# jhuldr/BrainFM

Hardware: AMD Instinct MI355X
Metric: voxels/sec whole-volume multi-task inference, 256^3 tiled (higher is better)
Workload: dtype f16x3-split (fp32-grade); 1 GPU; 256^3 volume, reference tiling win160/stride80 -> 27 tiles, UNet3D f64 x6 levels, 9 heads (69 ch), fused tail + deformed atlas + on-device stitch of 17 keys; stitched_keys=17, mfma_passes=3, submission=hipGraph replay per tile shape, parallelism=tiles sharded over 1 rank(s), gather to rank 0, tiles_in_flight_per_gpu=2

## Files before the change

### brainfm_amd/_lib.py

```python
import ctypes as C
import os

_HERE = os.path.dirname(os.path.abspath(__file__))
LIB_PATH = os.path.join(_HERE, "libbrainfm_hip.so")

ERR = {0: "BFM_OK", -1: "BFM_E_ARG", -2: "BFM_E_SHAPE", -3: "BFM_E_WORKSPACE", -4: "BFM_E_LAUNCH"}

ROLE_PLAIN, ROLE_CT, ROLE_BIAS_LOG, ROLE_SEG, ROLE_DIST, ROLE_SR, ROLE_PATHOL = range(7)
(EW_EXP, EW_AFFINE, EW_CLAMP, EW_CLAMP_MIN, EW_GAMMA, EW_SIGMOID, EW_DIV, EW_NONZERO, EW_SUB_DIV, EW_GE,
 EW_NAN_TO_NUM) = range(11)
(EW_ADD, EW_MUL, EW_MUL_EXP, EW_AXPY_CLAMP0, EW_AXPY, EW_DIV2, EW_ZERO_WHERE_ZERO) = range(7)


class BfmError(RuntimeError):
    pass


class Upsample(C.Structure):
    _fields_ = [("d", C.c_int), ("h", C.c_int), ("w", C.c_int),
                ("mapD", C.c_void_p), ("mapH", C.c_void_p), ("mapW", C.c_void_p),
                ("repD", C.c_void_p), ("repH", C.c_void_p), ("repW", C.c_void_p)]


CLASS_STATS_BLOCKS = 1024
# ... 94 lines not shown
    "bfm_conv3x3x3_upfold_batch_workspace": (_Z, [_I, _I, _I, _I, _I, _I]),
    "bfm_conv3x3x3_upfold_batch": (_I, [_P, _I, _I, _I, _I, _I, _P, _P, _P, _I, _P, _I, _I, _I, _P, _P, _Z, _I, _P]),
    "bfm_conv3x3x3_tap_batch_workspace": (_Z, [_I, _I, _I, _I]),
    "bfm_conv3x3x3_tap_batch": (_I, [_P, _I, _I, _I, _P, _P, _P, _I, _P, _I, _I, _I, _I, _I, _P, _Z, _I, _P]),
    "bfm_tap_sum_rows": (_I, [_I, _I]),
    "bfm_tap_sum_batch": (_I, [_P, _I, _I, _I, _I, _P, _I, _F, _I, _I, _P, _P, _P]),
    "bfm_moment_rows_bytes": (_Z, [_I, _I]),
    "bfm_conv3x3x3_mfma_rows": (_I, [_I, _I, _I, _I, _I, C.POINTER(_I)]),
    "bfm_conv3x3x3_mfma_ex": (_I, [_P, _I, _P, _I, _I, _I, _I, _UP, _P, _P, _P, _I, _P, _I, _I, _F, _I,
                                   C.POINTER(_I), _P, _P, _Z, _P, _P]),
    "bfm_conv3x3x3_mfma_batch_workspace": (_Z, [_I, _I, _I, _I, _I, _I, _I]),
    "bfm_conv3x3x3_mfma_batch": (_I, [_P, _I, _P, _I, _I, _I, _I, _I, _UP, _P, _P, _P, _I, _P, _I, _I, _F, _I,
                                      C.POINTER(_I), _P, _P, _Z, _P, _I, _P]),
    "bfm_gn_stats_batch_workspace": (_Z, [_I, _I, _I, _I, _I, _I, _UP]),
    "bfm_gn_stats_batch": (_I, [_P, _I, _P, _I, _I, _I, _I, _I, _UP, _P, _P, _I, _F, _P, _P, _P, _P, _Z, _P]),
    "bfm_gn_stats_rows_batch": (_I, [_P, _I, _I, _P, _I, _I, C.c_double, _L, _I, _P, _P, _I, _F, _P, _P, _P, _P]),
    "bfm_conv3x3x3_stem_rows": (_I, [_I, _I, _I]),
    "bfm_conv3x3x3_stem_ex": (_I, [_P, _I, _I, _I, _P, _P, _P, _P, _I, _F, _P, _P, _P]),
    "bfm_conv3x3x3_stem_mc_ex": (_I, [_P, _I, _I, _I, _I, _P, _P, _P, _P, _I, _F, _P, _P, _P]),
    "bfm_gn_stats_rows_workspace": (_Z, [_I, _I, _I, _I]),
    "bfm_gn_stats_plan": (_I, [_I, _L, _I, C.POINTER(_I), C.POINTER(_I), C.POINTER(_L), C.POINTER(_I)]),
    "bfm_gn_stats_rows_route": (_I, [_I, _I, _I, _I, _I, _I]),
    "bfm_gn_stats_rows": (_I, [_P, _I, _I, _P, _I, _I, C.c_double, _L, _P, _P, _I, _F, _P, _P, _P, _P, _Z, _P, _P]),
    "bfm_gn_stats_rows_sliced": (_I, [_P, _I, _I, _I, _I, _P, _I, _I, _I, _I, C.c_double, _L, _P, _P, _I, _F, _P, _P, _P, _P, _Z,
                                      _P, _P]),
    "bfm_gn_stats_rows_train": (_I, [_P, _I, _I, _P, _I, _I, C.c_double, _L, _P, _P, _I, _F, _P, _P, _P, _P, _P, _P, _Z, _P, _P]),
    "bfm_crop3d": (_I, [_P, _I, _I, _I, _I, _I, _I, _I, _I, _I, _P, _P]),
    "bfm_pack_conv_weights_wino4_bytes": (_Z, [_I, _I, _I]),
    "bfm_pack_conv_weights_wino4": (_I, [_P, _I, _I, _F, _I, _P, C.POINTER(_I), _P]),
    "bfm_conv3x3x3_wino4_rows": (_I, [_I, _I, _I, _I]),
    "bfm_conv3x3x3_wino4_box": (_I, [_I, _I, _I, _I, _P]),
    "bfm_conv3x3x3_wino4_masked_workspace": (_Z, [_I, _I, _I, _I]),
    "bfm_conv3x3x3_wino4_uniform_scratch": (_Z, [_I]),
    "bfm_conv3x3x3_wino4_uniform": (_I, [_P, _I, _I, _I, _I, _P, _P, _P, _I, _P, _I, _I, _F, _I, _I, _P, _P, _P, _P, _P]),
    "bfm_conv3x3x3_wino4_uniform_keep": (_I, [_P, _I, _I, _I, _I, _P, _P, _P, _I, _P, _I, _I, _F, _I, _I, _P, _P, _P, _P, _P, _P]),
    "bfm_conv3x3x3_wino4": (_I, [_P, _I, _I, _I, _I, _P, _P, _P, _I, _P, _I, _I, _F, _I, _I, _P, _P, _P]),
    "bfm_conv3x3x3_wino4_batch": (_I, [_P, _I, _I, _I, _I, _I, _P, _P, _P, _I, _P, _I, _I, _F, _I, _I, _P, _P, _I, _P]),
    "bfm_conv3x3x3_wino_b5_rows": (_I, [_I, _I, _I, _I]),
    "bfm_conv3x3x3_wino_b5_splitk": (_I, [_I, _I, _I, _I, _I]),
    "bfm_conv3x3x3_wino_b5_workspace": (_Z, [_I, _I, _I, _I, _I, _I]),
    "bfm_conv3x3x3_wino_b5_batch": (_I, [_P, _I, _I, _I, _I, _I, _P, _P, _P, _I, _P, _I, _I, _F, _I, _I, _P, _P, _I, _P, _Z,
                                         _P]),
    "bfm_conv3x3x3_wino4_masked": (_I, [_P, _I, _I, _I, _I, _P, _P, _P, _I, _P, _I, _I, _F, _I, _I, _P, _P, _P, _Z, _P]),
    "bfm_permute_flip3d": (_I, [_P, _I, _I, _I, C.POINTER(_I), C.POINTER(_I), _P, _P]),
    "bfm_bbox_nonzero": (_I, [_P, _I, _I, _I, _F, _P, _P]),
    "bfm_mean_lastdim": (_I, [_P, _L, _I, _P, _P]),
    "bfm_pack_conv_weights_wino_bytes": (_Z, [_I, _I, _I]),
    "bfm_pack_conv_weights_wino": (_I, [_P, _I, _I, _F, _I, _P, C.POINTER(_I), _P]),
    "bfm_bspline3_prefilter_axis": (_I, [_P, _I, _I, _I, _I, _I, _F, _F, _P, _F, _F, _F, _I, _P]),
    "bfm_bspline3_resample_axis": (_I, [_P, _I, _I, _I, _I, _P, _I, _I, _P, _P]),
    "bfm_conv3x3x3_wino_rows": (_I, [_I, _I, _I, _I]),
    "bfm_conv3x3x3_wino_ex": (_I, [_P, _I, _I, _I, _I, _P, _P, _P, _I, _P, _I, _I, _F, _I, _I, _P, _P, _P]),
    "bfm_conv3x3x3_wino_box": (_I, [_I, _I, _I, _I, _P]),
    "bfm_uniform_boxes": (_I, [_P, _I, _I, _I, _I, _I, _P, _P]),
    "bfm_uniform_boxes_level": (_I, [_P, _I, _I, _I, _I, _I, _I, _P, _P]),
    "bfm_uniform_boxes_levels": (_I, [_P, _I, _I, _I, _I, C.POINTER(_I), C.POINTER(_I), _I, C.POINTER(_P), _P, _P]),
    "bfm_uniform_boxes_bytes": (_Z, [_I, _I, _I, _I]),
    "bfm_uniform_fill": (_I, [_P, _I, _I, _I, _I, _I, _P, _P]),
    "bfm_conv3x3x3_wino_uniform_scratch": (_Z, [_I]),
    "bfm_conv3x3x3_wino_uniform": (_I, [_P, _I, _I, _I, _I, _P, _P, _P, _I, _P, _I, _I, _F, _I, _I, _P, _P, _P, _P, _P]),
    "bfm_conv3x3x3_wino_pool_ok": (_I, [_I, _I, _I, _I]),
    "bfm_conv3x3x3_wino_pool": (_I, [_P, _I, _I, _I, _I, _P, _P, _P, _I, _P, _I, _I, _F, _I, _I, _P, _P, _P, _P, _P]),
    "bfm_conv3x3x3_wino_uniform_pool": (_I, [_P, _I, _I, _I, _I, _P, _P, _P, _I, _P, _I, _I, _F, _I, _I, _P, _P, _P, _P, _P, _P,
                                             _P]),
    "bfm_conv3x3x3_wino_masked_workspace": (_Z, [_I, _I, _I, _I]),
    "bfm_conv3x3x3_wino_masked": (_I, [_P, _I, _I, _I, _I, _P, _P, _P, _I, _P, _I, _I, _F, _I, _I, _P, _P, _P, _Z, _P]),
# ... 259 lines not shown
```

### brainfm_amd/csrc/conv3d_wino4.hip

```cpp
#include "wino_shared.h"
#include <cstdlib>
#include <type_traits>

namespace {

typedef _Float16 half8 __attribute__((ext_vector_type(8)));
typedef float floatx16 __attribute__((ext_vector_type(16)));
typedef __fp16 fp16x2_t __attribute__((ext_vector_type(2)));

constexpr int KC = 16;
constexpr int NPOS = 6;
constexpr int NTHR = 256;
constexpr int NRG = NTHR / 32;
constexpr int MLD = 33;

struct W4Params {
    const float* A;
    int CA, D, H, W;
    const float *scale, *shift, *bound;
    int G;
    const uint4* wp;
    int wexp, Cout;
    float slope;
    float* out;
    int accum;
    int TD, TH, TW, HT, QW;
    int qw_shift, thq_shift;
    int nTy, nTx, nMt, NT, KCN;
    int npos_lds, plane_stride;
    double *rsum, *rsq;
    float *rmn, *rmx;
    const int* list;
    const int* list_n;
// ... 350 lines not shown
        if (p.rsum != nullptr) {
            double* ls = reinterpret_cast<double*>(lds + (size_t)NPOS * 64 * MLD * sizeof(float));
            double* lq = ls + NRG * 32;
            float* lmn = reinterpret_cast<float*>(lq + NRG * 32);
            float* lmx = lmn + NRG * 32;
            ls[rg * 32 + col] = (double)fs; lq[rg * 32 + col] = (double)fq;
            lmn[rg * 32 + col] = fmn; lmx[rg * 32 + col] = fmx;
            __syncthreads();
            if (tid < 32) {
                double Ssum = 0.0, Q = 0.0;
                float MN = INFINITY, MX = -INFINITY;
#pragma unroll
                for (int r = 0; r < NRG; ++r) {
                    Ssum += ls[r * 32 + tid]; Q += lq[r * 32 + tid];
                    MN = fminf(MN, lmn[r * 32 + tid]); MX = fmaxf(MX, lmx[r * 32 + tid]);
                }
                const size_t o = (size_t)mt * p.Cout + nt * 64 + nb * 32 + tid;
                p.rsum[o] = Ssum; p.rsq[o] = Q; p.rmn[o] = MN; p.rmx[o] = MX;
            }
        }
    }
}

template <int NPASS>
__global__ void __launch_bounds__(NTHR, 2) conv_wino4(const W4Params p) { conv_wino4_body<NPASS, 0>(p); }
template <int NPASS>
__global__ void __launch_bounds__(NTHR, 2) conv_wino4_masked(const W4Params p) { conv_wino4_body<NPASS, 1>(p); }

constexpr int DB_TD = 8, DB_TH = 8, DB_HT = 10, DB_NROW = 100;
constexpr int DB_PLANE = DB_NROW * 16;
constexpr int DB_RAWROW = 6 * 64;
constexpr int DB_RAW = DB_NROW * DB_RAWROW;
constexpr int DB_NDMA = DB_NROW / 2;
constexpr int DB_NDMA_WAVE = (DB_NDMA + 3) / 4;

template <bool LO>
__device__ __forceinline__ void split_store4_mix(const float (&t)[4], unsigned char* dp, int plane_stride) {
    const fp16x2_t h01 = __builtin_amdgcn_cvt_pkrtz(t[0], t[1]);
    const fp16x2_t h23 = __builtin_amdgcn_cvt_pkrtz(t[2], t[3]);
    uint2 hv;
    hv.x = __builtin_bit_cast(unsigned, h01);
    hv.y = __builtin_bit_cast(unsigned, h23);
    *reinterpret_cast<uint2*>(dp) = hv;
    if constexpr (LO) {
        uint2 lv;
        asm("v_fma_mixlo_f16 %0, %1, -1.0, %2 op_sel_hi:[1,0,0]" : "=v"(lv.x) : "v"(hv.x), "v"(t[0]));
        asm("v_fma_mixhi_f16 %0, %1, -1.0, %2 op_sel:[1,0,0] op_sel_hi:[1,0,0]" : "+v"(lv.x) : "v"(hv.x), "v"(t[1]));
        asm("v_fma_mixlo_f16 %0, %1, -1.0, %2 op_sel_hi:[1,0,0]" : "=v"(lv.y) : "v"(hv.y), "v"(t[2]));
        asm("v_fma_mixhi_f16 %0, %1, -1.0, %2 op_sel:[1,0,0] op_sel_hi:[1,0,0]" : "+v"(lv.y) : "v"(hv.y), "v"(t[3]));
        *reinterpret_cast<uint2*>(dp + plane_stride) = lv;
    }
}

template <int NPASS, int MODE, int ABL = 0>
__device__ __forceinline__ void conv_wino4d_body(const W4Params& pin) {
    W4Params p = pin;
    constexpr bool LIST = MODE != 0;
    constexpr bool UNI = MODE == 3;
    constexpr bool BY_FLAG = MODE == 2 || MODE == 3;
    constexpr int NPL = (NPASS == 3) ? 2 : 1;
    constexpr int NF = 2 * NPL;
    constexpr int NWF = 3 * NPL;
    constexpr int RAW_OFF = 2 * NPOS * NPL * DB_PLANE;
    extern __shared__ __attribute__((aligned(16))) unsigned char lds[];

    const int tid = threadIdx.x;
    const int lane = tid & 63;
    const int wv = __builtin_amdgcn_readfirstlane(tid >> 6);
    const int posA = wv;
    const int posB = 4 + (wv >> 1), nbB = wv & 1;
    const int l32 = lane & 31, khalf = lane >> 5;
#ifdef BFM_W4_ABLATE
    if (p.dbg_sleep > 0 && blockIdx.x < 512) {
        unsigned hwid;
        asm volatile("s_getreg_b32 %0, hwreg(HW_REG_HW_ID)" : "=s"(hwid));
        if (hwid & 1)
            for (int i = 0; i < p.dbg_sleep; ++i) __builtin_amdgcn_s_sleep(16);
    }
#endif
    int item;
    {
        const int nblk = LIST ? p.list_n[0] * p.NT : p.nMt * p.NT;
        const int bid = blockIdx.x;
        if (LIST && bid >= nblk) return;
        const int q = nblk >> 3, r = nblk & 7;
        const int xcd = bid & 7, idx = bid >> 3;
        item = (xcd < r ? xcd * (q + 1) : r * (q + 1) + (xcd - r) * q) + idx;
    }
    const int mt = LIST ? p.list[item / p.NT] : item / p.NT;
    const int nt = item % p.NT;
    int mtl = mt;
    if (!LIST && p.nMtS > 0) {
        const int smp = mt / p.nMtS;
        mtl = mt - smp * p.nMtS;
        p.A += smp * p.sA;
        p.out += smp * p.sO;
        p.scale += smp * p.saff;
        p.shift += smp * p.saff;
        p.bound += smp * p.G;
    }
    const int tx = mtl % p.nTx;
    const int ty = (mtl / p.nTx) % p.nTy;
    const int tz = mtl / (p.nTx * p.nTy);
    const int z0 = tz * DB_TD, y0 = ty * DB_TH, x0 = tx * 4;
    int cls = 0;
    if constexpr (BY_FLAG) cls = __builtin_amdgcn_readfirstlane((int)p.uni_flags[mt]);
    const bool rep = MODE == 2 && cls != 0;
    float4* const ybuf = BY_FLAG && cls ? reinterpret_cast<float4*>(p.uni_acc) + ((size_t)(cls - 1) * p.NT + nt) * (2 * 8 * NTHR) + tid
                                        : nullptr;
    bool store = true;
    if constexpr (UNI) {
        if (p.uni_need != nullptr) {
            store = p.uni_need[mt] != 0;
            if (!store && p.uni_keep != nullptr) store = p.uni_keep[((int64_t)z0 * p.H + y0) * p.W + x0] != 0.f;
        }
    }

    float bmax = 0.f;
    for (int g = 0; g < p.G; ++g) bmax = fmaxf(bmax, p.bound[g]);
    int aexp = 0;
    if (bmax > 0.f && bmax < INFINITY) {
        int ex;
        (void)frexpf(bmax, &ex);
        aexp = 10 - ex;
        aexp = aexp > 60 ? 60 : (aexp < -60 ? -60 : aexp);
    }
    const float a_scale = ldexpf(1.0f, aexp);
    const float dq = ldexpf(1.0f, -(aexp + p.wexp));

    floatx16 acc[2][2];
    floatx16 accB[2];
    if constexpr (!UNI) {
    int a_off[4];
#pragma unroll
    for (int u = 0; u < 4; ++u) {
        const int pos = u < 2 ? posA : posB, mb = u & 1;
        const int pr = row_perm(l32);
        const int d = mb * 2 + (pr >> 4) + 4 * ((pr & 15) >> 3), h = pr & 7;
        a_off[u] = ((pos * 2 + khalf) * NPL) * DB_PLANE + (d * DB_HT + h) * 16;
    }

    const int q4 = tid & 3;
    int msk[2];
#pragma unroll
    for (int it = 0; it < 2; ++it) {
        const int r = (tid >> 2) + 64 * it;
        msk[it] = -1;
        if (r < DB_NROW) {
            const int hz = r / DB_HT, hy = r - hz * DB_HT;
            const int gz = z0 + hz - 1, gy = y0 + hy - 1;
            int m = 0;
            if (gz >= 0 && gz < p.D && gy >= 0 && gy < p.H) {
#pragma unroll
                for (int i = 0; i < 6; ++i)
                    if (x0 - 1 + i >= 0 && x0 - 1 + i < p.W) m |= 1 << i;
            }
            msk[it] = m;
        }
    }
    const bool inner = z0 >= 1 && z0 + DB_TD < p.D && y0 >= 1 && y0 + DB_TH < p.H && x0 >= 1 && x0 + 4 < p.W;
    const int st_plane = ((q4 >> 1) * NPL) * DB_PLANE + (q4 & 1) * 8;

    const int slot = lane >> 2;
    const int sb = slot >= 6 ? 1 : 0;
    int gxc = x0 + (slot - 6 * sb) - 1;
    gxc = gxc < 0 ? 0 : (gxc > p.W - 1 ? p.W - 1 : gxc);
    const int lane_el = gxc * p.CA + (lane & 3) * 4;
    const bool dma_lane = slot < 12;
    const unsigned raw_lds = (unsigned)(__UINTPTR_TYPE__)((__attribute__((address_space(3))) unsigned char*)(lds + RAW_OFF));
    const int zs = z0 > 0 ? z0 - 1 : 0;
    const float* slab = p.A + (int64_t)zs * p.H * p.W * p.CA;
    auto issue_dma = [&](int kc) __attribute__((always_inline)) {
        if constexpr ((ABL & 8) != 0) return;
        if (dma_lane) {
            int wvo = wv;
            asm volatile("" : "+s"(wvo));
#pragma unroll
            for (int n = 0; n < DB_NDMA_WAVE; ++n) {
                const int i = wvo + 4 * n;
                if (n < DB_NDMA_WAVE - 1 || i < DB_NDMA) {
                    const int hz = i / 5, hp = i - 5 * hz;
                    int gz = z0 + hz - 1;
                    gz = gz < 0 ? 0 : (gz > p.D - 1 ? p.D - 1 : gz);
                    int gy0 = y0 + 2 * hp - 1, gy1 = gy0 + 1;
                    gy0 = gy0 < 0 ? 0 : (gy0 > p.H - 1 ? p.H - 1 : gy0);
                    gy1 = gy1 > p.H - 1 ? p.H - 1 : gy1;
                    const unsigned ro0 = (unsigned)((((gz - zs) * p.H + gy0) * p.W) * p.CA);
                    const unsigned ro1 = (unsigned)((((gz - zs) * p.H + gy1) * p.W) * p.CA);
                    const unsigned vo = ((sb ? ro1 : ro0) + (unsigned)lane_el) * 4u;
                    const unsigned la = raw_lds + (unsigned)(i * (2 * DB_RAWROW));
                    asm volatile("s_mov_b32 m0, %2\n\ts_nop 0\n\tglobal_load_lds_dwordx4 %0, %1" ::"v"(vo), "s"(slab + kc * KC), "s"(la)
                                 : "memory");
                }
            }
        }
    };

#pragma unroll
    for (int u = 0; u < 2; ++u) {
#pragma unroll
        for (int i = 0; i < 16; ++i) { acc[u][0][i] = 0.f; acc[u][1][i] = 0.f; accB[u][i] = 0.f; }
    }

    const int S = p.KCN * 9;
    const uint4* wbA = p.wp + (size_t)(nt * NPOS + posA) * S * (NF * 64) + lane;
    const uint4* wbB = p.wp + (size_t)(nt * NPOS + posB) * S * (NF * 64) + nbB * (NPL * 64) + lane;
    uint4 wq[3][NWF];
    auto fetch = [&](int s, uint4 (&dst)[NWF]) __attribute__((always_inline)) {
        if constexpr ((ABL & 1) != 0) { if (s > 2) return; }
        const int sc = s < S ? s : S - 1;
#pragma unroll
        for (int f = 0; f < NF; ++f) dst[f] = wbA[(size_t)sc * (NF * 64) + f * 64];
#pragma unroll
        for (int f = 0; f < NPL; ++f) dst[NF + f] = wbB[(size_t)sc * (NF * 64) + f * 64];
    };
    issue_dma(0);
    fetch(0, wq[0]);
    fetch(1, wq[1]);
    half8 a_abl[4][NPL];
    if constexpr ((ABL & 2) != 0) {
#pragma unroll
        for (int u = 0; u < 4; ++u)
#pragma unroll
            for (int hl = 0; hl < NPL; ++hl)
#pragma unroll
                for (int j = 0; j < 8; ++j) a_abl[u][hl][j] = (_Float16)(0.01f * (float)((lane * 7 + u * 3 + hl * 5 + j) % 61) - 0.3f);
    }

    for (int kc = 0; kc < p.KCN; ++kc) {
        const int c0 = kc * KC;
        const float4 sc4 = *reinterpret_cast<const float4*>(p.scale + c0 + q4 * 4);
        const float4 sh4 = *reinterpret_cast<const float4*>(p.shift + c0 + q4 * 4);
        const float sc[4] = {sc4.x * a_scale, sc4.y * a_scale, sc4.z * a_scale, sc4.w * a_scale};
        const float sh[4] = {sh4.x * a_scale, sh4.y * a_scale, sh4.z * a_scale, sh4.w * a_scale};
        __builtin_amdgcn_s_waitcnt(0x0F70);
        __syncthreads();
#pragma unroll
        for (int it = 0; it < 2; ++it) {
            if (msk[it] < 0) continue;
            if constexpr ((ABL & 4) != 0) continue;
            const int r = (tid >> 2) + 64 * it;
            const float4* rp = reinterpret_cast<const float4*>(
                __builtin_assume_aligned(lds + RAW_OFF + r * DB_RAWROW + q4 * 16, 16));
            float4 v[6];
#pragma unroll
            for (int i = 0; i < 6; ++i) v[i] = rp[i * 4];
            float dd[6][4];
            if (inner) {
#pragma unroll
                for (int i = 0; i < 6; ++i) {
                    const float y[4] = {v[i].x, v[i].y, v[i].z, v[i].w};
#pragma unroll
                    for (int c = 0; c < 4; ++c) dd[i][c] = fmaf(y[c], sc[c], sh[c]);
                }
            } else {
#pragma unroll
                for (int i = 0; i < 6; ++i) {
                    const bool ok = msk[it] & (1 << i);
                    const float y[4] = {v[i].x, v[i].y, v[i].z, v[i].w};
#pragma unroll
                    for (int c = 0; c < 4; ++c) {
                        const float a = fmaf(y[c], sc[c], sh[c]);
                        dd[i][c] = ok ? a : 0.f;
                    }
                }
            }
            unsigned char* dst = lds + st_plane + r * 16;
            float t[6][4];
#pragma unroll
            for (int c = 0; c < 4; ++c) {
                const float d0 = dd[0][c], d1 = dd[1][c], d2 = dd[2][c], d3 = dd[3][c], d4 = dd[4][c], d5 = dd[5][c];
                const float a = fmaf(-4.f, d2, d4);
                const float b = fmaf(-4.f, d1, d3);
                const float cc = d4 - d2;
// ... 43 lines not shown
                    for (int nb = 0; nb < 2; ++nb) {
                        const half8 bhi = __builtin_bit_cast(half8, wq[cur][nb * NPL]);
                        if constexpr (NPASS == 3) {
                            const half8 blo = __builtin_bit_cast(half8, wq[cur][nb * NPL + 1]);
                            acc[u][nb] = __builtin_amdgcn_mfma_f32_32x32x16_f16(a[1], bhi, acc[u][nb], 0, 0, 0);
                            acc[u][nb] = __builtin_amdgcn_mfma_f32_32x32x16_f16(a[0], blo, acc[u][nb], 0, 0, 0);
                        }
                        acc[u][nb] = __builtin_amdgcn_mfma_f32_32x32x16_f16(a[0], bhi, acc[u][nb], 0, 0, 0);
                    }
                } else {
                    const half8 bhi = __builtin_bit_cast(half8, wq[cur][NF]);
                    if constexpr (NPASS == 3) {
                        const half8 blo = __builtin_bit_cast(half8, wq[cur][NF + 1]);
                        accB[u - 2] = __builtin_amdgcn_mfma_f32_32x32x16_f16(a[1], bhi, accB[u - 2], 0, 0, 0);
                        accB[u - 2] = __builtin_amdgcn_mfma_f32_32x32x16_f16(a[0], blo, accB[u - 2], 0, 0, 0);
                    }
                    accB[u - 2] = __builtin_amdgcn_mfma_f32_32x32x16_f16(a[0], bhi, accB[u - 2], 0, 0, 0);
                }
            }
        }
    }

    }

    if constexpr ((ABL & 16) != 0) {
        float sm = 0.f;
#pragma unroll
        for (int u = 0; u < 2; ++u)
#pragma unroll
            for (int i = 0; i < 16; ++i) sm += acc[u][0][i] + acc[u][1][i] + accB[u][i];
        if (sm == 12345.678f) p.out[tid] = sm;
        return;
    }
    float* m = reinterpret_cast<float*>(lds);
    const int col = tid & 31, rg = tid >> 5;
    const bool interior = z0 + DB_TD <= p.D && y0 + DB_TH <= p.H && x0 + 4 <= p.W;
    int un[4];
#pragma unroll
    for (int c = 0; c < 4; ++c) un[c] = row_unperm(16 * (c >> 1) + 8 * (c & 1) + rg);
    const unsigned off_t = (unsigned)((rg * p.W) * p.Cout + col);
#pragma unroll
    for (int nb = 0; nb < 2; ++nb) {
        if constexpr (!UNI && (ABL & 256) == 0) {
        __syncthreads();
#pragma unroll
        for (int u = 0; u < 2; ++u) {
            float* mw = m + (posA * 64 + u * 32 + khalf * 4) * MLD + l32;
#pragma unroll
            for (int i = 0; i < 16; ++i)
                mw[((i >> 2) * 8 + (i & 3)) * MLD] = acc[u][nb][i];
        }
        if (nbB == nb) {
#pragma unroll
            for (int u = 0; u < 2; ++u) {
                float* mw = m + (posB * 64 + u * 32 + khalf * 4) * MLD + l32;
#pragma unroll
                for (int i = 0; i < 16; ++i)
                    mw[((i >> 2) * 8 + (i & 3)) * MLD] = accB[u][i];
            }
        }
        __syncthreads();
        } else if (nb == 1 && p.rsum != nullptr) __syncthreads();
        float fs = 0.f, fq = 0.f, fmn = INFINITY, fmx = -INFINITY;
        float* ob = p.out + nt * 64 + nb * 32 + ((int64_t)(z0 * p.H + y0) * p.W + x0) * p.Cout;
        if constexpr ((ABL & 512) != 0) ob = p.out + nt * 64 + nb * 32 + (mt & 127) * 16384;
        const float* mc = m + col;
        if (interior) {
// ... 46 lines not shown
#pragma unroll 2
            for (int it = 0; it < 8; ++it) {
                if (z0 + it >= p.D) break;
                float* o = ob + (int64_t)it * p.H * p.W * p.Cout;
                float y[4];
                if constexpr (UNI) {
                    const float4 yy = ybuf[(nb * 8 + it) * NTHR];
                    y[0] = yy.x; y[1] = yy.y; y[2] = yy.z; y[3] = yy.w;
                } else {
                    const int qr = 32 * ((it & 3) >> 1) + row_unperm(16 * (it & 1) + 8 * (it >> 2) + rg);
                    const float* mr = mc + qr * MLD;
                    const float m0 = mr[0 * 64 * MLD], m1 = mr[1 * 64 * MLD], m2 = mr[2 * 64 * MLD];
                    const float m3 = mr[3 * 64 * MLD], m4 = mr[4 * 64 * MLD], m5 = mr[5 * 64 * MLD];
                    const float s1 = m1 + m2, d1 = m1 - m2, s2 = m3 + m4, d2 = m3 - m4;
                    y[0] = ((m0 + s1) + s2) * dq;
                    y[1] = fmaf(2.f, d2, d1) * dq;
                    y[2] = fmaf(4.f, s2, s1) * dq;
                    y[3] = (fmaf(8.f, d2, d1) + m5) * dq;
                    if (MODE == 2 && rep) ybuf[(nb * 8 + it) * NTHR] = make_float4(y[0], y[1], y[2], y[3]);
                }
#pragma unroll
                for (int k = 0; k < 4; ++k) {
                    if (x0 + k < p.W) {
                        float r = y[k];
                        if (p.accum) r = r + o[off_t + (unsigned)(k * p.Cout)];
                        r = r >= 0.f ? r : r * p.slope;
                        if (!UNI || store) o[off_t + (unsigned)(k * p.Cout)] = r;
                        fs += r; fq = fmaf(r, r, fq); fmn = fminf(fmn, r); fmx = fmaxf(fmx, r);
                    }
                }
            }
        }
        if (p.rsum != nullptr) {
            double* ls = reinterpret_cast<double*>(lds + (UNI ? (size_t)0 : (size_t)NPOS * 64 * MLD * sizeof(float)));
            double* lq = ls + NRG * 32;
            float* lmn = reinterpret_cast<float*>(lq + NRG * 32);
            float* lmx = lmn + NRG * 32;
            ls[rg * 32 + col] = (double)fs; lq[rg * 32 + col] = (double)fq;
            lmn[rg * 32 + col] = fmn; lmx[rg * 32 + col] = fmx;
            __syncthreads();
            if (tid < 32) {
                double Ssum = 0.0, Q = 0.0;
                float MN = INFINITY, MX = -INFINITY;
#pragma unroll
                for (int r = 0; r < NRG; ++r) {
                    Ssum += ls[r * 32 + tid]; Q += lq[r * 32 + tid];
                    MN = fminf(MN, lmn[r * 32 + tid]); MX = fmaxf(MX, lmx[r * 32 + tid]);
                }
                const size_t o = (size_t)mt * p.Cout + nt * 64 + nb * 32 + tid;
                p.rsum[o] = Ssum; p.rsq[o] = Q; p.rmn[o] = MN; p.rmx[o] = MX;
            }
        }
    }
}

template <int NPASS>
__global__ void __launch_bounds__(NTHR, 2) conv_wino4d(const W4Params p) { conv_wino4d_body<NPASS, 0>(p); }
template <int NPASS>
__global__ void __launch_bounds__(NTHR, 2) conv_wino4d_masked(const W4Params p) { conv_wino4d_body<NPASS, 1>(p); }
template <int NPASS>
__global__ void __launch_bounds__(NTHR, 2) conv_wino4d_rest(const W4Params p) { conv_wino4d_body<NPASS, 2>(p); }
template <int NPASS>
__global__ void __launch_bounds__(NTHR, 2) conv_wino4d_uniform(const W4Params p) { conv_wino4d_body<NPASS, 3>(p); }
#ifdef BFM_W4_ABLATE
template <int ABL>
__global__ void __launch_bounds__(NTHR, 2) conv_wino4d_abl(const W4Params p) { conv_wino4d_body<3, 0, ABL>(p); }
#endif

__global__ void pack_wino4(const float* __restrict__ w, int Cin, int Cout, int wexp, int npl, uint4* __restrict__ out) {
    const int KCN = Cin / KC;
    const int nf = 2 * npl;
    const int64_t n = (int64_t)(Cout / 64) * NPOS * KCN * 9 * nf * 64;
    const double s = ldexp(1.0, wexp);
    for (int64_t i = (int64_t)blockIdx.x * blockDim.x + threadIdx.x; i < n; i += (int64_t)gridDim.x * blockDim.x) {
        const int lane = (int)(i & 63);
        int64_t r = i >> 6;
        const int f = (int)(r % nf); r /= nf;
        const int t = (int)(r % 9); r /= 9;
        const int kc = (int)(r % KCN); r /= KCN;
        const int ps = (int)(r % NPOS); r /= NPOS;
        const int ntile = (int)r;
        const int nb = f / npl, hl = f - nb * npl;
        const int co = ntile * 64 + nb * 32 + (lane & 31);
        const int ci0 = kc * KC + 8 * (lane >> 5);
        half8 v;
#pragma unroll
        for (int j = 0; j < 8; ++j) {
            const float* g = w + ((size_t)co * Cin + ci0 + j) * 27 + t * 3;
            const double g0 = g[0], g1 = g[1], g2 = g[2];
            const double u = ps == 0 ? g0 / 4.0
                           : ps == 1 ? -((g0 + g1) + g2) / 6.0
                           : ps == 2 ? -((g0 - g1) + g2) / 6.0
                           : ps == 3 ? g0 / 24.0 + g1 / 12.0 + g2 / 6.0
                           : ps == 4 ? g0 / 24.0 - g1 / 12.0 + g2 / 6.0
                                     : g2;
            const float x = (float)(u * s);
            const _Float16 hh = (_Float16)x;
            v[j] = hl == 0 ? hh : (_Float16)(x - (float)hh);
        }
        out[i] = __builtin_bit_cast(uint4, v);
    }
}

int ilog2i(int v) { int r = 0; while ((1 << r) < v) ++r; return r; }

bool choose_box4(int D, int H, int W, int npl, int& TD, int& TH, int& TW) {
    if (!bfm_wino_choose_box(D, H, W, npl, TD, TH, TW)) return false;
    if (TW % 4 || TD * TH * (TW / 4) != 64) return false;
    const int64_t npos = (int64_t)(TD + 2) * (TH + 2) * (TW / 4);
    if (npos * 4 > 3 * NTHR) return false;
    const int64_t plane = ((npos * 16 + 255) / 256) * 256 + 16;
    return 2 * NPOS * npl * plane <= 62 * 1024;
}

bool use_dma_kernel(int D, int H, int W) {
#ifdef BFM_W4_ABLATE
    if (getenv("BFM_W4_OLD")) return false;
#endif
    return D >= DB_TD && H >= DB_TH && W >= 4;
}

bool choose_box_any(int D, int H, int W, int npl, int& TD, int& TH, int& TW) {
    if (use_dma_kernel(D, H, W)) { TD = DB_TD; TH = DB_TH; TW = 4; return true; }
    return choose_box4(D, H, W, npl, TD, TH, TW);
}

}

extern "C" size_t bfm_pack_conv_weights_wino4_bytes(int Cin, int Cout, int passes) {
    if (Cin <= 0 || Cout <= 0 || Cin % KC || Cout % 64) return 0;
    const int npl = passes == 3 ? 2 : 1;
    return (size_t)(Cout / 64) * NPOS * (Cin / KC) * 9 * 2 * npl * 64 * sizeof(uint4);
}

extern "C" int bfm_pack_conv_weights_wino4(const float* w_oidhw, int Cin, int Cout, float wmax_abs_host, int passes,
                                           void* wpacked, int* wexp_host, bfm_stream_t stream) {
    if (!w_oidhw || !wpacked || !wexp_host || Cin <= 0 || Cout <= 0) return BFM_E_ARG;
    if (Cin % KC || Cout % 64 || (passes != 1 && passes != 3)) return BFM_E_SHAPE;
    int wexp = 0;
    if (wmax_abs_host > 0.f && wmax_abs_host < INFINITY) {
        int ex;
        (void)frexpf(wmax_abs_host, &ex);
        wexp = 14 - ex;
        wexp = wexp > 60 ? 60 : (wexp < -60 ? -60 : wexp);
    }
    *wexp_host = wexp;
    const int npl = passes == 3 ? 2 : 1;
    const int64_t n = (int64_t)(Cout / 64) * NPOS * (Cin / KC) * 9 * 2 * npl * 64;
    const int nb = (int)std::min<int64_t>(8192, bfm_cdiv64(n, 256));
    hipLaunchKernelGGL(pack_wino4, dim3(nb), dim3(256), 0, bfm_s(stream), w_oidhw, Cin, Cout, wexp, npl,
                       static_cast<uint4*>(wpacked));
    return bfm_launch_status();
}

extern "C" int bfm_conv3x3x3_wino4_rows(int D, int H, int W, int passes) {
    int TD, TH, TW;
    if (D <= 0 || H <= 0 || W <= 0 || !choose_box_any(D, H, W, passes == 3 ? 2 : 1, TD, TH, TW)) return 0;
    return (int)bfm_box_count(D, H, W, TD, TH, TW);
}

extern "C" int bfm_conv3x3x3_wino4_box(int D, int H, int W, int passes, int* box) {
    int TD, TH, TW;
    if (!box || D <= 0 || H <= 0 || W <= 0 || !choose_box_any(D, H, W, passes == 3 ? 2 : 1, TD, TH, TW)) return BFM_E_ARG;
    box[0] = TD; box[1] = TH; box[2] = TW;
    return BFM_OK;
}

extern "C" size_t bfm_conv3x3x3_wino4_masked_workspace(int D, int H, int W, int passes) {
    const int n = bfm_conv3x3x3_wino4_rows(D, H, W, passes);
    if (n <= 0) return 0;
    return MaskListBuf::bytes((size_t)n);
}

static int w4_launch(const WinoLaunch& a) {
    if (const int rc = bfm_wino_check(a, KC)) return rc;
    const int D = a.D, H = a.H, W = a.W, CA = a.CA, Cout = a.Cout, passes = a.passes;
    const int S = a.batch.S, affine_stride = a.batch.affine_stride;
    const int npl = passes == 3 ? 2 : 1;
    W4Params p{};
    p.A = a.A; p.CA = CA; p.D = D; p.H = H; p.W = W;
    p.scale = a.scale; p.shift = a.shift; p.bound = a.bound; p.G = a.G;
    p.wp = static_cast<const uint4*>(a.wpacked);
    p.wexp = a.wexp; p.Cout = Cout; p.slope = a.slope; p.out = a.out; p.accum = a.flags & 1;
    if (!choose_box_any(D, H, W, npl, p.TD, p.TH, p.TW)) return BFM_E_SHAPE;
    const bool dma = use_dma_kernel(D, H, W);
    if (dma && (int64_t)(DB_TD + 2) * H * W * CA >= (int64_t)1 << 30) return BFM_E_SHAPE;
    p.HT = p.TH + 2; p.QW = p.TW / 4;
    p.qw_shift = ilog2i(p.QW); p.thq_shift = ilog2i(p.TH * p.QW);
    const int nTz = bfm_cdiv(D, p.TD);
    p.nTy = bfm_cdiv(H, p.TH); p.nTx = bfm_cdiv(W, p.TW);
    p.nMt = nTz * p.nTy * p.nTx;
    if (S > 1 || affine_stride > 0) {
        if (a.mask.img || S < 1 || (affine_stride != 0 && (affine_stride < CA || (affine_stride & 3)))) return BFM_E_ARG;
        p.nMtS = p.nMt;
        p.nMt = S * p.nMtS;
        p.saff = affine_stride > 0 ? affine_stride : CA;
        p.sA = (int64_t)D * H * W * CA;
        p.sO = (int64_t)D * H * W * Cout;
    }
    p.NT = Cout / 64;
    p.KCN = CA / KC;
    p.npos_lds = (p.TD + 2) * p.HT * p.QW;
    p.plane_stride = ((p.npos_lds * 16 + 255) / 256) * 256 + 16;
    size_t smem = dma ? (size_t)2 * NPOS * npl * DB_PLANE + DB_RAW : (size_t)2 * NPOS * npl * p.plane_stride;
    const size_t epi = (size_t)NPOS * 64 * MLD * sizeof(float) + (size_t)NRG * 32 * 24;
    if (smem < epi) smem = epi;
    if (smem > (dma ? 80u : 64u) * 1024) return BFM_E_SHAPE;
    const UniformFlagBuf fb{a.uniform.flags, (size_t)p.nMt};
    if (fb.flags) {
        int bd, bh, bw;
        if (!dma || a.mask.img || S > 1 || affine_stride > 0 || !a.uniform.scratch) return BFM_E_ARG;
        if (!bfm_wino_choose_box(D, H, W, npl, bd, bh, bw) || bd != p.TD || bh != p.TH || bw != p.TW) return BFM_E_SHAPE;
        p.uni_flags = fb.flags;
        p.uni_acc = a.uniform.scratch;
        if (a.uniform.keep && !(a.flags & 2)) return BFM_E_ARG;
        if ((a.flags & 3) == 3) { p.uni_need = fb.need(); p.uni_keep = a.uniform.keep; }
    }
    if (dma) {
        static bool attr = false;
        if (const int rc = bfm_raise_lds_limit(
                attr,
                {bfm_kernel(&conv_wino4d_rest<3>), bfm_kernel(&conv_wino4d_rest<1>), bfm_kernel(&conv_wino4d<3>),
                 bfm_kernel(&conv_wino4d<1>), bfm_kernel(&conv_wino4d_masked<3>), bfm_kernel(&conv_wino4d_masked<1>)},
                80 * 1024))
            return rc;
    }
    MomentRows rows;
    if (a.moment_rows && !rows.carve(a.moment_rows, (size_t)p.nMt * Cout)) return BFM_E_ARG;
    rows.into(p);
    if ((int64_t)p.nMt * p.NT > 0x7fffffff) return BFM_E_SHAPE;
    const dim3 grid((unsigned)(p.nMt * p.NT)), block(NTHR);
    hipStream_t st = bfm_s(a.stream);
    if (a.mask.img) {
        if (!a.mask.ws) return BFM_E_ARG;
        const MaskListBuf mb{a.mask.ws, (size_t)p.nMt};
        if (const int rc = bfm_wino_mask_list(a.mask.img, D, H, W, p.TD, p.TH, p.TW, p.nTy, p.nTx, p.nMt, a.mask.ws, a.stream))
            return rc;
        p.list = mb.list(); p.list_n = mb.count();
        if (dma) bfm_launch_by_passes(passes, conv_wino4d_masked<3>, conv_wino4d_masked<1>, grid, block, smem, st, p);
        else bfm_launch_by_passes(passes, conv_wino4_masked<3>, conv_wino4_masked<1>, grid, block, smem, st, p);
        return bfm_launch_status();
    }
    if (fb.flags) {
        p.list = fb.rest_list(); p.list_n = fb.counts();
        bfm_launch_by_passes(passes, conv_wino4d_rest<3>, conv_wino4d_rest<1>, grid, block, smem, st, p);
        p.list = fb.uniform_list(); p.list_n = fb.counts() + 1;
        bfm_launch_by_passes(passes, conv_wino4d_uniform<3>, conv_wino4d_uniform<1>, grid, block, 6144, st, p);
        return bfm_launch_status();
    }
#ifdef BFM_W4_ABLATE
    if (const char* e = getenv("BFM_W4_SLEEP")) p.dbg_sleep = atoi(e);
    if (const char* e = getenv("BFM_W4_ABL")) {
        const int abl = atoi(e);
        if (dma) {
#define W4D_ATTR(N) (void)hipFuncSetAttribute(reinterpret_cast<const void*>(&conv_wino4d_abl<N>), hipFuncAttributeMaxDynamicSharedMemorySize, 80 * 1024)
            W4D_ATTR(0); W4D_ATTR(1); W4D_ATTR(2); W4D_ATTR(3); W4D_ATTR(4); W4D_ATTR(8); W4D_ATTR(12); W4D_ATTR(15); W4D_ATTR(16); W4D_ATTR(31); W4D_ATTR(64); W4D_ATTR(28); W4D_ATTR(128); W4D_ATTR(256); W4D_ATTR(384); W4D_ATTR(512);
            switch (abl) {
#define W4D_CASE(N) case N: hipLaunchKernelGGL(conv_wino4d_abl<N>, grid, dim3(NTHR), smem, st, p); return bfm_launch_status()
                W4D_CASE(0); W4D_CASE(1); W4D_CASE(2); W4D_CASE(3); W4D_CASE(4); W4D_CASE(8); W4D_CASE(12); W4D_CASE(15); W4D_CASE(16); W4D_CASE(31); W4D_CASE(64); W4D_CASE(28); W4D_CASE(128); W4D_CASE(256); W4D_CASE(384); W4D_CASE(512);
                default: return BFM_E_ARG;
            }
        }
    }
#endif
    if (dma) bfm_launch_by_passes(passes, conv_wino4d<3>, conv_wino4d<1>, grid, block, smem, st, p);
    else bfm_launch_by_passes(passes, conv_wino4<3>, conv_wino4<1>, grid, block, smem, st, p);
    return bfm_launch_status();
}

extern "C" int bfm_conv3x3x3_wino4(const float* A, int CA, int D, int H, int W, const float* scale, const float* shift,
                                   const float* bound, int G, const void* wpacked, int wexp, int Cout, float slope,
                                   int passes, int flags, float* out, void* moment_rows, bfm_stream_t stream) {
    return w4_launch({A, CA, D, H, W, scale, shift, bound, G, wpacked, wexp, Cout, slope, passes, flags, out, moment_rows, stream});
}

extern "C" int bfm_conv3x3x3_wino4_batch(const float* A, int CA, int S, int D, int H, int W, const float* scale,
                                         const float* shift, const float* bound, int G, const void* wpacked, int wexp,
                                         int Cout, float slope, int passes, int flags, float* out, void* moment_rows,
                                         int affine_stride, bfm_stream_t stream) {
    if (S < 1) return BFM_E_ARG;
    WinoLaunch a{A, CA, D, H, W, scale, shift, bound, G, wpacked, wexp, Cout, slope, passes, flags, out, moment_rows, stream};
    a.batch = {S, affine_stride > 0 ? affine_stride : CA};
    return w4_launch(a);
}

extern "C" int bfm_conv3x3x3_wino4_masked(const float* A, int CA, int D, int H, int W, const float* scale, const float* shift,
                                          const float* bound, int G, const void* wpacked, int wexp, int Cout, float slope,
                                          int passes, int flags, float* out, const float* mask_image, void* workspace,
                                          size_t workspace_bytes, bfm_stream_t stream) {
    if (!mask_image || (flags & ~1)) return BFM_E_ARG;
    if (!workspace || (reinterpret_cast<uintptr_t>(workspace) & 3) ||
        workspace_bytes < bfm_conv3x3x3_wino4_masked_workspace(D, H, W, passes))
        return BFM_E_ARG;
    WinoLaunch a{A, CA, D, H, W, scale, shift, bound, G, wpacked, wexp, Cout, slope, passes, flags, out, nullptr, stream};
    a.mask = {mask_image, workspace};
    return w4_launch(a);
}

// ... 29 lines not shown
```

### include/brainfm_hip.h

```cpp
#ifndef BRAINFM_HIP_H
#define BRAINFM_HIP_H

#include <stddef.h>
#include <stdint.h>

#ifdef __cplusplus
extern "C" {
#endif

typedef void* bfm_stream_t;

#define BFM_OK 0
#define BFM_E_ARG (-1)
#define BFM_E_SHAPE (-2)
#define BFM_E_WORKSPACE (-3)
#define BFM_E_LAUNCH (-4)

typedef struct {
    int d, h, w;
    const int32_t* mapD; const int32_t* mapH; const int32_t* mapW;
    const int32_t* repD; const int32_t* repH; const int32_t* repW;
} bfm_upsample_t;

const char* bfm_version(void);
// ... 99 lines not shown
                          const float* bound, const float* wpacked_direct, int Cout, float slope, float* out,
                          void* moment_rows , bfm_stream_t stream);
int bfm_conv3x3x3_stem_mc_ex(const float* A, int Cin, int D, int H, int W, const float* scale, const float* shift,
                             const float* bound, const float* wpacked_direct, int Cout, float slope, float* out,
                             void* moment_rows , bfm_stream_t stream);
size_t bfm_gn_stats_rows_workspace(int nrowsA, int CA, int nrowsB, int CB);
#define BFM_GN_TICKETS 16
#define BFM_GN_ROWS_DIRECT 0
#define BFM_GN_ROWS_FOLD 1
#define BFM_GN_ROWS_ONE_LAUNCH 2
int bfm_gn_stats_rows_route(int nrowsA, int CA, int nrowsB, int CB, int G, int has_ticket);
int bfm_gn_stats_rows(const void* rowsA, int nrowsA, int CA, const void* rowsB, int nrowsB, int CB, double weightB,
                      int64_t nvox, const float* gamma, const float* beta, int G, float eps, float* scale,
                      float* shift, float* bound, void* workspace, size_t workspace_bytes, void* ticket,
                      bfm_stream_t stream);
int bfm_gn_stats_rows_train(const void* rowsA, int nrowsA, int CA, const void* rowsB, int nrowsB, int CB, double weightB,
                            int64_t nvox, const float* gamma, const float* beta, int G, float eps, float* scale,
                            float* shift, float* bound, float* mean_out, float* rstd_out, void* workspace,
                            size_t workspace_bytes, void* ticket, bfm_stream_t stream);

int bfm_gn_stats_rows_sliced(const void* rowsA, int totalA, int firstA, int nrowsA, int CA, const void* rowsB, int totalB,
                             int firstB, int nrowsB, int CB, double weightB, int64_t nvox, const float* gamma,
                             const float* beta, int G, float eps, float* scale, float* shift, float* bound,
                             void* workspace, size_t workspace_bytes, void* ticket, bfm_stream_t stream);

size_t bfm_pack_conv_weights_wino4_bytes(int Cin, int Cout, int passes);
int bfm_pack_conv_weights_wino4(const float* w_oidhw, int Cin, int Cout, float wmax_abs_host, int passes, void* wpacked,
                                int* wexp_host, bfm_stream_t stream);
int bfm_conv3x3x3_wino4_rows(int D, int H, int W, int passes);
int bfm_conv3x3x3_wino4_box(int D, int H, int W, int passes, int* box );
int bfm_conv3x3x3_wino4(const float* A, int CA, int D, int H, int W, const float* scale, const float* shift,
                        const float* bound, int G, const void* wpacked, int wexp, int Cout, float slope, int passes,
                        int flags, float* out, void* moment_rows , bfm_stream_t stream);
int bfm_conv3x3x3_wino4_batch(const float* A, int CA, int S, int D, int H, int W, const float* scale, const float* shift,
                              const float* bound, int G, const void* wpacked, int wexp, int Cout, float slope, int passes,
                              int flags, float* out, void* moment_rows, int affine_stride, bfm_stream_t stream);
int bfm_conv3x3x3_wino_b5_rows(int D, int H, int W, int passes);
int bfm_conv3x3x3_wino_b5_splitk(int Cin, int Cout, int D, int H, int W);
size_t bfm_conv3x3x3_wino_b5_workspace(int Cin, int Cout, int S, int D, int H, int W);
int bfm_conv3x3x3_wino_b5_batch(const float* A, int CA, int S, int D, int H, int W, const float* scale, const float* shift,
                                const float* bound, int G, const void* wpacked, int wexp, int Cout, float slope, int passes,
                                int flags, float* out, void* moment_rows, int affine_stride, void* workspace,
                                size_t workspace_bytes, bfm_stream_t stream);
size_t bfm_conv3x3x3_wino4_masked_workspace(int D, int H, int W, int passes);
size_t bfm_conv3x3x3_wino4_uniform_scratch(int Cout);
int bfm_conv3x3x3_wino4_uniform(const float* A, int CA, int D, int H, int W, const float* scale, const float* shift,
                                const float* bound, int G, const void* wpacked, int wexp, int Cout, float slope, int passes,
                                int flags, float* out, void* moment_rows, const unsigned char* uniform_flags, void* scratch,
                                bfm_stream_t stream);
int bfm_conv3x3x3_wino4_uniform_keep(const float* A, int CA, int D, int H, int W, const float* scale, const float* shift,
                                     const float* bound, int G, const void* wpacked, int wexp, int Cout, float slope,
                                     int passes, int flags, float* out, void* moment_rows, const unsigned char* uniform_flags,
                                     void* scratch, const float* keep_image, bfm_stream_t stream);
int bfm_conv3x3x3_wino4_masked(const float* A, int CA, int D, int H, int W, const float* scale, const float* shift,
                               const float* bound, int G, const void* wpacked, int wexp, int Cout, float slope, int passes,
                               int flags, float* out, const float* mask_image, void* workspace, size_t workspace_bytes,
                               bfm_stream_t stream);

size_t bfm_conv3x3x3_mfma_workspace(int Cin, int Cout, int D, int H, int W, int splitk);
int bfm_conv3x3x3_mfma_plan(int Cin, int Cout, int D, int H, int W, int* cfg_out );

size_t bfm_pack_conv_weights_upfold_bytes(int CB, int Cout, int passes);
int bfm_pack_conv_weights_upfold(const float* w_oidhw , int CA, int CB, int Cout,
                                 float wmax_abs_host, int passes, void* wpacked, int* wexp_host, bfm_stream_t stream);
int bfm_conv3x3x3_upfold(const float* B, int CB, int d, int h, int w, const float* scale_b, const float* shift_b,
                         const float* bound, int G, const void* wpacked, int wexp, int Cout, int passes, float* out,
// ... 506 lines not shown
```

Before: 220.6 million voxels/s.

## Add paired-workgroup wino4 conv kernel sharing one input staging for two N tiles

Adds a 512-thread variant of the DMA wino4 conv in which two 256-thread halves compute adjacent output-channel tiles while sharing a single LDS-staged input box. The DMA and transform work is split across eight waves instead of four, and each half keeps its own epilogue region in LDS. This is meant to halve the input loads and transforms per output tile and to improve the wave-quantization tail. A heuristic enables it when Cout is a multiple of 128 and the last wave of blocks is at least 180 of 256 CUs, and an env var or API call can override that. In exchange it drops to one workgroup per CU and needs more LDS.

```diff
diff --git a/brainfm_amd/_lib.py b/brainfm_amd/_lib.py
--- a/brainfm_amd/_lib.py
+++ b/brainfm_amd/_lib.py
@@ -150,6 +150,7 @@
     "bfm_conv3x3x3_wino4_box": (_I, [_I, _I, _I, _I, _P]),
     "bfm_conv3x3x3_wino4_masked_workspace": (_Z, [_I, _I, _I, _I]),
     "bfm_conv3x3x3_wino4_uniform_scratch": (_Z, [_I]),
+    "bfm_conv3x3x3_wino4_set_pair": (_I, [_I]),
     "bfm_conv3x3x3_wino4_uniform": (_I, [_P, _I, _I, _I, _I, _P, _P, _P, _I, _P, _I, _I, _F, _I, _I, _P, _P, _P, _P, _P]),
     "bfm_conv3x3x3_wino4_uniform_keep": (_I, [_P, _I, _I, _I, _I, _P, _P, _P, _I, _P, _I, _I, _F, _I, _I, _P, _P, _P, _P, _P, _P]),
     "bfm_conv3x3x3_wino4": (_I, [_P, _I, _I, _I, _I, _P, _P, _P, _I, _P, _I, _I, _F, _I, _I, _P, _P, _P]),
diff --git a/brainfm_amd/csrc/conv3d_wino4.hip b/brainfm_amd/csrc/conv3d_wino4.hip
--- a/brainfm_amd/csrc/conv3d_wino4.hip
+++ b/brainfm_amd/csrc/conv3d_wino4.hip
@@ -1,4 +1,5 @@
 #include "wino_shared.h"
+#include <atomic>
 #include <cstdlib>
 #include <type_traits>
 
@@ -415,7 +416,7 @@
 constexpr int DB_RAWROW = 6 * 64;
 constexpr int DB_RAW = DB_NROW * DB_RAWROW;
 constexpr int DB_NDMA = DB_NROW / 2;
-constexpr int DB_NDMA_WAVE = (DB_NDMA + 3) / 4;
+constexpr int DB_EPI = NPOS * 64 * MLD * (int)sizeof(float) + NRG * 32 * 24;
 
 template <bool LO>
 __device__ __forceinline__ void split_store4_mix(const float (&t)[4], unsigned char* dp, int plane_stride) {
@@ -435,21 +436,28 @@
     }
 }
 
-template <int NPASS, int MODE, int ABL = 0>
+template <int NPASS, int MODE, int ABL = 0, bool PAIR = false>
 __device__ __forceinline__ void conv_wino4d_body(const W4Params& pin) {
     W4Params p = pin;
     constexpr bool LIST = MODE != 0;
     constexpr bool UNI = MODE == 3;
     constexpr bool BY_FLAG = MODE == 2 || MODE == 3;
+    static_assert(!PAIR || MODE == 0, "the pair form is the dense one");
     constexpr int NPL = (NPASS == 3) ? 2 : 1;
     constexpr int NF = 2 * NPL;
     constexpr int NWF = 3 * NPL;
     constexpr int RAW_OFF = 2 * NPOS * NPL * DB_PLANE;
+    constexpr int NWV = PAIR ? 8 : 4;
+    constexpr int NIT = PAIR ? 1 : 2;
+    constexpr int NDMA_WAVE = (DB_NDMA + NWV - 1) / NWV;
     extern __shared__ __attribute__((aligned(16))) unsigned char lds[];
 
-    const int tid = threadIdx.x;
+    const int tid_wg = threadIdx.x;
+    const int tid = PAIR ? (tid_wg & (NTHR - 1)) : tid_wg;
+    const int half = PAIR ? __builtin_amdgcn_readfirstlane(tid_wg >> 8) : 0;
     const int lane = tid & 63;
     const int wv = __builtin_amdgcn_readfirstlane(tid >> 6);
+    const int wv_wg = PAIR ? __builtin_amdgcn_readfirstlane(tid_wg >> 6) : wv;
     const int posA = wv;
     const int posB = 4 + (wv >> 1), nbB = wv & 1;
     const int l32 = lane & 31, khalf = lane >> 5;
@@ -461,17 +469,18 @@
             for (int i = 0; i < p.dbg_sleep; ++i) __builtin_amdgcn_s_sleep(16);
     }
 #endif
+    const int NTI = PAIR ? p.NT >> 1 : p.NT;
     int item;
     {
-        const int nblk = LIST ? p.list_n[0] * p.NT : p.nMt * p.NT;
+        const int nblk = LIST ? p.list_n[0] * NTI : p.nMt * NTI;
         const int bid = blockIdx.x;
         if (LIST && bid >= nblk) return;
         const int q = nblk >> 3, r = nblk & 7;
         const int xcd = bid & 7, idx = bid >> 3;
         item = (xcd < r ? xcd * (q + 1) : r * (q + 1) + (xcd - r) * q) + idx;
     }
-    const int mt = LIST ? p.list[item / p.NT] : item / p.NT;
-    const int nt = item % p.NT;
+    const int mt = LIST ? p.list[item / NTI] : item / NTI;
+    const int nt = PAIR ? 2 * (item % NTI) + half : item % NTI;
     int mtl = mt;
     if (!LIST && p.nMtS > 0) {
         const int smp = mt / p.nMtS;
@@ -524,10 +533,10 @@
     }
 
     const int q4 = tid & 3;
-    int msk[2];
-#pragma unroll
-    for (int it = 0; it < 2; ++it) {
-        const int r = (tid >> 2) + 64 * it;
+    int msk[NIT];
+#pragma unroll
+    for (int it = 0; it < NIT; ++it) {
+        const int r = (tid_wg >> 2) + 64 * it;
         msk[it] = -1;
         if (r < DB_NROW) {
             const int hz = r / DB_HT, hy = r - hz * DB_HT;
@@ -556,12 +565,12 @@
     auto issue_dma = [&](int kc) __attribute__((always_inline)) {
         if constexpr ((ABL & 8) != 0) return;
         if (dma_lane) {
-            int wvo = wv;
+            int wvo = wv_wg;
             asm volatile("" : "+s"(wvo));
 #pragma unroll
-            for (int n = 0; n < DB_NDMA_WAVE; ++n) {
-                const int i = wvo + 4 * n;
-                if (n < DB_NDMA_WAVE - 1 || i < DB_NDMA) {
+            for (int n = 0; n < NDMA_WAVE; ++n) {
+                const int i = wvo + NWV * n;
+                if (n < NDMA_WAVE - 1 || i < DB_NDMA) {
                     const int hz = i / 5, hp = i - 5 * hz;
                     int gz = z0 + hz - 1;
                     gz = gz < 0 ? 0 : (gz > p.D - 1 ? p.D - 1 : gz);
@@ -619,10 +628,10 @@
         __builtin_amdgcn_s_waitcnt(0x0F70);
         __syncthreads();
 #pragma unroll
-        for (int it = 0; it < 2; ++it) {
+        for (int it = 0; it < NIT; ++it) {
             if (msk[it] < 0) continue;
             if constexpr ((ABL & 4) != 0) continue;
-            const int r = (tid >> 2) + 64 * it;
+            const int r = (tid_wg >> 2) + 64 * it;
             const float4* rp = reinterpret_cast<const float4*>(
                 __builtin_assume_aligned(lds + RAW_OFF + r * DB_RAWROW + q4 * 16, 16));
             float4 v[6];
@@ -732,7 +741,8 @@
         if (sm == 12345.678f) p.out[tid] = sm;
         return;
     }
-    float* m = reinterpret_cast<float*>(lds);
+    unsigned char* const lds_epi = PAIR ? lds + half * DB_EPI : lds;
+    float* m = reinterpret_cast<float*>(lds_epi);
     const int col = tid & 31, rg = tid >> 5;
     const bool interior = z0 + DB_TD <= p.D && y0 + DB_TH <= p.H && x0 + 4 <= p.W;
     int un[4];
@@ -845,7 +855,7 @@
             }
         }
         if (p.rsum != nullptr) {
-            double* ls = reinterpret_cast<double*>(lds + (UNI ? (size_t)0 : (size_t)NPOS * 64 * MLD * sizeof(float)));
+            double* ls = reinterpret_cast<double*>(lds_epi + (UNI ? (size_t)0 : (size_t)NPOS * 64 * MLD * sizeof(float)));
             double* lq = ls + NRG * 32;
             float* lmn = reinterpret_cast<float*>(lq + NRG * 32);
             float* lmx = lmn + NRG * 32;
@@ -875,6 +885,8 @@
 __global__ void __launch_bounds__(NTHR, 2) conv_wino4d_rest(const W4Params p) { conv_wino4d_body<NPASS, 2>(p); }
 template <int NPASS>
 __global__ void __launch_bounds__(NTHR, 2) conv_wino4d_uniform(const W4Params p) { conv_wino4d_body<NPASS, 3>(p); }
+template <int NPASS>
+__global__ void __launch_bounds__(2 * NTHR, 1) conv_wino4d_pair(const W4Params p) { conv_wino4d_body<NPASS, 0, 0, true>(p); }
 #ifdef BFM_W4_ABLATE
 template <int ABL>
 __global__ void __launch_bounds__(NTHR, 2) conv_wino4d_abl(const W4Params p) { conv_wino4d_body<3, 0, ABL>(p); }
@@ -938,6 +950,28 @@
     return choose_box4(D, H, W, npl, TD, TH, TW);
 }
 
+int pair_mode_from_env() {
+    const char* e = getenv("BFM_W4_PAIR");
+    if (!e || !e[0]) return 1;
+    if (e[0] == 'f' || e[0] == 'F') return 2;
+    const int v = atoi(e);
+    return v < 0 ? 0 : (v > 2 ? 2 : v);
+}
+std::atomic<int>& pair_mode() {
+    static std::atomic<int> m{pair_mode_from_env()};
+    return m;
+}
+
+constexpr int W4_CUS = 256;
+constexpr int W4_PAIR_MIN_TAIL = 180;
+bool use_pair_kernel(int Cout, int64_t boxes) {
+    const int mode = pair_mode().load(std::memory_order_relaxed);
+    if (mode == 0 || Cout % 128) return false;
+    if (mode == 2) return true;
+    const int64_t tail = (boxes * (Cout / 128) - 1) % W4_CUS + 1;
+    return tail >= W4_PAIR_MIN_TAIL;
+}
+
 }
 
 extern "C" size_t bfm_pack_conv_weights_wino4_bytes(int Cin, int Cout, int passes) {
@@ -983,6 +1017,11 @@
     const int n = bfm_conv3x3x3_wino4_rows(D, H, W, passes);
     if (n <= 0) return 0;
     return MaskListBuf::bytes((size_t)n);
+}
+
+extern "C" int bfm_conv3x3x3_wino4_set_pair(int mode) {
+    if (mode < 0 || mode > 2) return pair_mode().load();
+    return pair_mode().exchange(mode);
 }
 
 static int w4_launch(const WinoLaunch& a) {
@@ -1038,11 +1077,21 @@
                 80 * 1024))
             return rc;
     }
+    const bool pair = dma && !a.mask.img && !fb.flags && use_pair_kernel(Cout, p.nMt);
+    const size_t smem_pair = std::max(smem, (size_t)2 * DB_EPI);
+    if (pair) {
+        static bool attr_pair = false;
+        if (const int rc = bfm_raise_lds_limit(
+                attr_pair,
+                {bfm_kernel(&conv_wino4d_pair<3>), bfm_kernel(&conv_wino4d_pair<1>)}, (int)smem_pair))
+            return rc;
+    }
     MomentRows rows;
     if (a.moment_rows && !rows.carve(a.moment_rows, (size_t)p.nMt * Cout)) return BFM_E_ARG;
     rows.into(p);
     if ((int64_t)p.nMt * p.NT > 0x7fffffff) return BFM_E_SHAPE;
     const dim3 grid((unsigned)(p.nMt * p.NT)), block(NTHR);
+    const dim3 grid_pair((unsigned)(p.nMt * (p.NT / 2))), block_pair(2 * NTHR);
     hipStream_t st = bfm_s(a.stream);
     if (a.mask.img) {
         if (!a.mask.ws) return BFM_E_ARG;
@@ -1076,7 +1125,8 @@
         }
     }
 #endif
-    if (dma) bfm_launch_by_passes(passes, conv_wino4d<3>, conv_wino4d<1>, grid, block, smem, st, p);
+    if (pair) bfm_launch_by_passes(passes, conv_wino4d_pair<3>, conv_wino4d_pair<1>, grid_pair, block_pair, smem_pair, st, p);
+    else if (dma) bfm_launch_by_passes(passes, conv_wino4d<3>, conv_wino4d<1>, grid, block, smem, st, p);
     else bfm_launch_by_passes(passes, conv_wino4<3>, conv_wino4<1>, grid, block, smem, st, p);
     return bfm_launch_status();
 }
diff --git a/include/brainfm_hip.h b/include/brainfm_hip.h
--- a/include/brainfm_hip.h
+++ b/include/brainfm_hip.h
@@ -155,6 +155,7 @@
 int bfm_conv3x3x3_wino4(const float* A, int CA, int D, int H, int W, const float* scale, const float* shift,
                         const float* bound, int G, const void* wpacked, int wexp, int Cout, float slope, int passes,
                         int flags, float* out, void* moment_rows , bfm_stream_t stream);
+int bfm_conv3x3x3_wino4_set_pair(int mode);
 int bfm_conv3x3x3_wino4_batch(const float* A, int CA, int S, int D, int H, int W, const float* scale, const float* shift,
                               const float* bound, int G, const void* wpacked, int wexp, int Cout, float slope, int passes,
                               int flags, float* out, void* moment_rows, int affine_stride, bfm_stream_t stream);
```

New measurement: 221.6 million voxels/s (median of 6 runs). No clear change (+0.4%).
